# automl/TransformersCanDoBayesianInference

Hardware: AMD Instinct MI355X
Metric: synthetic datasets/sec (GP prior, bptt=2000) (higher is better)
Workload: dtype fp16; 1 GPU; priors.fast_gp, bptt=2000, num_features=18, emsize=512, nhead=4, nhid=1024, nlayers=6, 1000 bars (BASELINE.json configs[1]); per_gpu_batch=64, global_batch=64, aggregate_k_gradients=1, aggregate_streams=0, aggregate_stacked=False, seq_len=2000, parallelism=dp1, micro_batch_streams=2, eval_pos=weighted sampler(2000)

## Files before the change

### include/pfn_hip.h

```cpp
#ifndef PFN_HIP_H
#define PFN_HIP_H

#include <stddef.h>
#include <stdint.h>

#ifdef __cplusplus
extern "C" {
#endif

#define PFN_ABI_VERSION 10

enum {
  PFN_OK = 0,
  PFN_ERR_UNSUPPORTED = -1,
  PFN_ERR_ALIGNMENT = -2,
  PFN_ERR_LAUNCH = -3,
  PFN_ERR_ARGUMENT = -4,
};

enum { PFN_PREC_BF16 = 0,
       PFN_PREC_F32 = 1,
       PFN_PREC_FP16 = 2   };

typedef struct pfn_model_desc {
// ... 24 lines not shown
       PFN_TUNE_GEMM_TN_WRAP = 1,
       PFN_TUNE_FUSE_LNBWD = 2,
       PFN_TUNE_ATTN_PINGPONG = 4,
       PFN_TUNE_FUSE_LN_WIDE = 5,
       PFN_TUNE_GP_PLANES = 8,
       PFN_TUNE_FUSE_DELTA = 9,
       PFN_TUNE_GEMM_LN_ROWS = 7,
       PFN_TUNE_ATTN_BWD_GROUP = 10,
       PFN_TUNE_WGRAD_SPLITS = 11,
       PFN_TUNE_WGRAD_WAVES = 14,
       PFN_TUNE_LOSS_SCALE_TARGET = 15,
       PFN_TUNE_RESIDUAL16 = 16,
       PFN_TUNE_FUSE_Q_PROJECTION = 12,
       PFN_TUNE_KEY_CENTERING = 13,
       PFN_TUNE_ATTN_CACHE_SPLITS = 17,
       PFN_TUNE_TOP_LAYER_TEST_ROWS = 6  };
int pfn_set_tuning(int key, int value);
enum { PFN_PROF_ATTN_FWD = 0, PFN_PROF_ATTN_BWD_DELTA = 2, PFN_PROF_ATTN_BWD_KV = 4, PFN_PROF_ATTN_BWD_DQ = 6, PFN_PROF_GEMM_QKV = 8,
       PFN_PROF_GEMM_OUT_LN = 10, PFN_PROF_GEMM_LIN1 = 12, PFN_PROF_GEMM_LIN2_LN = 14, PFN_PROF_GEMM_DHPRE = 16, PFN_PROF_GEMM_DY1 = 18,
       PFN_PROF_GEMM_DCTX = 20, PFN_PROF_GEMM_DX = 22, PFN_PROF_WGRAD = 24, PFN_PROF_SLOTS = 26 };
int pfn_profile_enable(int on);
int pfn_profile_read(int slot, double* total_ms, int64_t* launches);

int pfn_param_layout(const pfn_model_desc* d, int64_t* offsets, int64_t* numels, int max_tensors);
int64_t pfn_param_count(const pfn_model_desc* d);
int64_t pfn_shadow_bytes(const pfn_model_desc* d);
int pfn_prepare_params(const pfn_model_desc* d, const float* params, void* shadow, void* stream);

int64_t pfn_workspace_bytes(const pfn_model_desc* d, int B, int S);
int64_t pfn_top_layer_rows(const pfn_model_desc* d, int B, int S, int sep, int use_dropout);
// ... 157 lines not shown
                      float* value, float* grad, void* stream);
int pfn_bnn_predict(const float* x_test, const float* theta, int64_t ld, int P, int K, int m, int F, int H, int activation,
                    float* prob1, void* stream);

int pfn_mlp_prior_forward(const float* weights, const float* biases, const int32_t* model_of, const int32_t* dims,
                          const float* noise_std, float* causes, const float* noise, float* y, float* hidden,
                          int B, int T, int HP, int Lmax, int activation, int gen_causes,
                          uint64_t seed, uint64_t offset, void* stream);

int pfn_op_gemm_nt(const void* A, int64_t lda, const void* B, int64_t ldb, int M, int N, int K,
                   int flags, const float* bias, const void* aux, int64_t ld_aux,
                   const float* resid, int64_t ld_resid, float* out_f32, int64_t ld_out_f32,
                   void* out_t, int64_t ld_out_t, void* out2_t, int64_t ld_out2, int prec, void* stream);
int pfn_op_gemm_tn(const void* A, int64_t lda, const void* B, int64_t ldb, float* C, int64_t ldc,
                   int M, int P, int Q, int atomic, int prec, void* stream);
int pfn_op_gemm_tn_group(int n, const void* const* A, const int64_t* lda, const void* const* B, const int64_t* ldb,
                         float* const* C, const int64_t* ldc, const int32_t* P, const int32_t* Q,
                         float* const* colsum, int M, int splits, int prec, void* stream);
#define PFN_OP_SUMS_16BIT 256
int pfn_op_gemm_ln(const void* A, int64_t lda, const void* B, int64_t ldb, int M, int N, int K, const float* bias,
                   const float* resid, const float* ry, const float* rmean, const float* rrstd,
                   const float* rgamma, const float* rbeta, const float* gamma, const float* beta, float eps,
                   float* y, float* mean, float* rstd, void* x_t, int prec, void* stream);
int pfn_op_gemm_lnbwd(const void* A, int64_t lda, const void* B, int64_t ldb, int M, int N, int K, const void* aux,
                      const float* y, const float* mean, const float* rstd, const float* gamma,
                      void* dx_t, float* dgamma, float* dbeta, int prec, void* stream);
int pfn_op_attention_fwd(const void* qkv, void* ctx, float* lse, int B, int S, int E, int H, int sep,
                         int prec, void* stream);
int64_t pfn_op_attention_bwd_ws_bytes(int B, int S, int H, int prec);
int pfn_op_attention_bwd(const void* qkv, const void* ctx, const float* lse, const void* dctx,
// ... 23 lines not shown
```

### transformerscandobayesianinference_amd/_hip.py

```python
import ctypes
import os
import subprocess

import torch

_HERE = os.path.dirname(os.path.abspath(__file__))
LIB_PATH = os.path.join(_HERE, 'libpfn_hip.so')
ABI_VERSION = 10

MAX_FEATURES = 1022
PREC_BF16 = 0
PREC_F32 = 1
PREC_FP16 = 2
PRECISIONS = {'bf16': PREC_BF16, 'f32': PREC_F32, 'fp32': PREC_F32, 'fp16': PREC_FP16, 'f16': PREC_FP16}
SCHED_TOP_LAYER_ALL_ROWS, SCHED_FUSE_LN_WIDE, SCHED_SEPARATE_LNBWD, SCHED_DETERMINISTIC, SCHED_NO_KEY_CENTERING, SCHED_FUSE_Q_PROJECTION, SCHED_KEY_CENTERING, SCHED_F32_RESIDUAL = 1, 2, 4, 8, 16, 32, 64, 128
NUTS_ADAPT_MASS, NUTS_KEEP_WARMUP, NUTS_MAX_WINDOWS, NUTS_INV_MASS_OFFSET = 1, 2, 16, 256

EPI_BIAS, EPI_GELU, EPI_GELU_BWD, EPI_RESID, EPI_OUT_F32, EPI_OUT_T, EPI_OUT2_T, EPI_ACCUM, EPI_RESID_T = 1, 2, 4, 8, 16, 32, 64, 128, 256


class HipExtensionError(RuntimeError):
    pass


# ... 55 lines not shown
    'pfn_clip_adam_step': (_I, [_P, _P, _P, _P, _L, _F, _F, _F, _F, _F, _F, _I, _I, _P, _P]),
    'pfn_gp_workspace_bytes': (_L, [_I, _I]),
    'pfn_gp_prior_sample': (_I, [_P, _P, _P, _P, _L, _P, _P, _P, _I, _I, _I, _I, _I, _I, _U64, _U64, _P, _P]),
    'pfn_gp_posterior': (_I, [_P, _P, _P, _L, _P, _P, _P, _P, _P, _I, _I, _I, _I, _P, _P, _P, _P, _P]),
    'pfn_gp_fit_workspace_bytes': (_L, [_I, _I]),
    'pfn_gp_mll_grad': (_I, [_P, _P, _P, _P, _P, _I, _I, _I, _I, _I, _P, _L, _P, _P, _P, _P]),
    'pfn_gp_fit_predict': (_I, [_P, _P, _P, _P, _P, _I, _I, _I, _I, _P, _I, _P, _L, _P, _P, _P, _P]),
    'pfn_nuts_workspace_bytes': (_L, [_I, _I, _I]),
    'pfn_nuts_init': (_I, [_P, _L, _I, _I, _L, _I, _I, _I, _I, _P, _I, _I, _F, _F, _U64, _P, _P, _P, _P, _P, _P]),
    'pfn_nuts_advance': (_I, [_P, _L, _I, _I, _L, _I, _I, _I, _P, _P, _P, _P, _P, _P, _P, _P, _P, _P, _P]),
    'pfn_bnn_logp_grad': (_I, [_P, _P, _P, _P, _L, _I, _I, _I, _I, _I, _I, _P, _P, _P]),
    'pfn_bnn_predict': (_I, [_P, _P, _L, _I, _I, _I, _I, _I, _I, _P, _P]),
    'pfn_mlp_prior_forward': (_I, [_P, _P, _P, _P, _P, _P, _P, _P, _P, _I, _I, _I, _I, _I, _I, _U64, _U64, _P]),
    'pfn_op_gemm_nt': (_I, [_P, _L, _P, _L, _I, _I, _I, _I, _P, _P, _L, _P, _L, _P, _L, _P, _L, _P, _L, _I, _P]),
    'pfn_op_gemm_tn': (_I, [_P, _L, _P, _L, _P, _L, _I, _I, _I, _I, _I, _P]),
    'pfn_op_gemm_tn_group': (_I, [_I, _P, _P, _P, _P, _P, _P, _P, _P, _P, _I, _I, _I, _P]),
    'pfn_op_gemm_ln': (_I, [_P, _L, _P, _L, _I, _I, _I, _P, _P, _P, _P, _P, _P, _P, _P, _P, _F, _P, _P, _P, _P, _I, _P]),
    'pfn_op_gemm_lnbwd': (_I, [_P, _L, _P, _L, _I, _I, _I, _P, _P, _P, _P, _P, _P, _P, _P, _I, _P]),
    'pfn_op_attention_fwd': (_I, [_P, _P, _P, _I, _I, _I, _I, _I, _I, _P]),
    'pfn_op_attention_bwd_ws_bytes': (_L, [_I, _I, _I, _I]),
    'pfn_op_attention_fwd_from': (_I, [_P, _P, _P, _I, _I, _I, _I, _I, _I, _I, _P]),
    'pfn_op_attention_bwd_from': (_I, [_P, _P, _P, _P, _P, _P, _P, _I, _I, _I, _I, _I, _I, _I, _I, _P]),
    'pfn_op_gather_rows': (_I, [_P, _P, _I, _I, _L, _I, _P]),
    'pfn_op_scatter_rows': (_I, [_P, _P, _I, _I, _L, _I, _I, _P]),
    'pfn_op_attention_bwd': (_I, [_P, _P, _P, _P, _P, _P, _P, _I, _I, _I, _I, _I, _I, _I, _P]),
    'pfn_op_layernorm_fwd': (_I, [_P, _P, _P, _P, _P, _P, _P, _L, _I, _F, _I, _P]),
    'pfn_op_layernorm_bwd': (_I, [_P, _I, _P, _P, _P, _P, _P, _P, _P, _P, _P, _L, _I, _I, _P]),
    'pfn_op_cast': (_I, [_P, _P, _L, _I, _P]),
    'pfn_op_qkv_projection': (_I, [_P, _P, _P, _P, _P, _I, _I, _I, _I, _P, _I, _I, _P]),
}
# ... 54 lines not shown
```

### transformerscandobayesianinference_amd/csrc/gemm_tn.hip

```cpp
#include <type_traits>
#include "pfn_device.h"
#include "pfn_kernels.h"

namespace pfn {

PFN_DEV int xcd_remap(int bid, int nwg) {
  const int q = nwg >> 3, r = nwg & 7, xcd = bid & 7;
  return (xcd < r ? xcd * (q + 1) : r * (q + 1) + (xcd - r) * q) + (bid >> 3);
}
typedef __attribute__((address_space(1))) const void gvoid_t;
typedef __attribute__((address_space(3))) void lvoid_t;

constexpr int TN_BMK = 32;

template <typename T>
__global__ __launch_bounds__(256, 2) void gemm_tn_kernel(GemmTN g) {
  constexpr int RB = 128 * sizeof(T);
  constexpr int TILE = TN_BMK * RB;
  extern __shared__ __attribute__((aligned(16))) char smem_raw[];
  LdsPtr smem = lds_cast(smem_raw);
  auto tileA = [&](int buf) { return smem + buf * 2 * TILE; };
  auto tileB = [&](int buf) { return smem + buf * 2 * TILE + TILE; };

  const int p0 = blockIdx.y * 128, q0 = blockIdx.x * 128;
// ... 473 lines not shown
#else
    return PFN_ERR_UNSUPPORTED;
#endif
  }
  static LdsAllowance allowance[2];
  if (precision == PFN_PREC_FP16) {
    allowance[1].ensure(gemm_tn_big_kernel<f16>, TNB_LDS);
    hipLaunchKernelGGL(gemm_tn_big_kernel<f16>, dim3(tiles * splits), dim3(512), TNB_LDS, stream, g);
  } else {
    allowance[0].ensure(gemm_tn_big_kernel<bf16>, TNB_LDS);
    hipLaunchKernelGGL(gemm_tn_big_kernel<bf16>, dim3(tiles * splits), dim3(512), TNB_LDS, stream, g);
  }
  return hipGetLastError() == hipSuccess ? PFN_OK : PFN_ERR_LAUNCH;
}

}
```

### transformerscandobayesianinference_amd/csrc/pfn_api.hip

```cpp
#include <algorithm>
#include <cstdarg>
#include <cstdio>
#include <cstring>
#include <mutex>
#include <vector>
#include "pfn_kernels.h"

using namespace pfn;

namespace pfn {
namespace {
struct ProfPair { hipEvent_t a, b; };
std::mutex g_prof_mu;
std::vector<ProfPair> g_prof[PFN_PROF_SLOTS];
std::atomic<int> g_prof_on{0};
}
bool prof_enabled() { return g_prof_on.load(std::memory_order_relaxed) != 0; }
void* prof_begin(int slot, hipStream_t s) {
  const int on = g_prof_on.load(std::memory_order_relaxed);
  if (!on || slot < 0 || slot >= PFN_PROF_SLOTS) return nullptr;
  if (on >= 2 && (slot & ~1) != on - 2) return nullptr;
  ProfPair* p = new ProfPair;
  if (hipEventCreate(&p->a) != hipSuccess || hipEventCreate(&p->b) != hipSuccess) { delete p; return nullptr; }
  (void)hipEventRecord(p->a, s);
// ... 93 lines not shown
  float* x0; char* x0_t;
  char* xaug_t;
  float* embacc;
  float* xaug_amax;
  std::vector<LayerWs> layer;
  char *xt_t, *dpre, *dt;
  char *dlog_t, *dd_t, *dctx_t;
  float *dxt, *gA, *delta;
  char* ds;
  char* gA_t;
  char *top_ctx_t, *top_dy1_t, *top_dctx_t;
  float *top_ry, *top_rmean, *top_rrstd;
  float* kshift;
  float* lscale;
  float* ln_part;
  int64_t bytes;
};

struct Ragged { const int32_t* sep_of; const int64_t* row_off; int64_t test_rows; int sep_min; };

static bool key_centering(const pfn_model_desc& d) {
  return (d.precision == PFN_PREC_FP16 && !(d.schedule & PFN_SCHED_NO_KEY_CENTERING)) || (d.precision == PFN_PREC_BF16 && (d.schedule & PFN_SCHED_KEY_CENTERING));
}

static bool residual16(const pfn_model_desc& d) {
  const int E = d.emsize;
  const bool wide = (d.schedule & PFN_SCHED_FUSE_LN_WIDE) != 0;
  return d.precision == PFN_PREC_FP16 && !(d.schedule & PFN_SCHED_F32_RESIDUAL) && d.nlayers > 0 && d.dropout == 0.f && d.nhid % 32 == 0 &&
         (E == 128 || E == 256 || E == 512 || (E == 1024 && wide));
}
static bool residual16_separate_ln(const pfn_model_desc& d, bool ln_fusable) {
  return d.precision == PFN_PREC_FP16 && !(d.schedule & PFN_SCHED_F32_RESIDUAL) && d.nlayers > 0 && d.dropout == 0.f && d.emsize >= 1024 && d.emsize % 8 == 0 && !ln_fusable;
}

Ws carve(const pfn_model_desc& d, int B, int S, char* base) {
  Ws w;
  const int64_t M = (int64_t)B * S, E = d.emsize, F = d.nhid, es = esize(d.precision);
  const int64_t npad = align_up(d.n_out, 8);
  int64_t cur = 0;
  auto take = [&](int64_t nbytes) { char* p = base ? base + cur : nullptr; cur = align_up(cur + nbytes, 256); return p; };
  w.x0 = (float*)take(M * E * 4); w.x0_t = take(M * E * es);
  const int64_t aug = emb_aug_width(d.num_features) > 0 ? emb_aug_width(d.num_features) : 32;
  w.xaug_t = take(M * aug * es); w.embacc = (float*)take(E * aug * 4);
  w.xaug_amax = (float*)take(aug * 4);
  w.layer.resize(d.nlayers);
  for (auto& l : w.layer) {
    l.qkv = take(M * 3 * E * es); l.ctx = take(M * E * es); l.lse = (float*)take((int64_t)B * d.nhead * S * 4);
    l.y1 = (float*)take(M * E * 4); l.mean1 = (float*)take(M * 4); l.rstd1 = (float*)take(M * 4);
    l.x1 = (float*)take(M * E * 4); l.x1_t = take(M * E * es);
// ... 4 lines not shown
    l.dy2m_t = l.dy1m_t = nullptr;
    if (d.dropout > 0.f) { l.dy2m_t = take(M * E * es); l.dy1m_t = take(M * E * es); }
  }
  w.xt_t = take(M * E * es); w.dpre = take(M * F * es); w.dt = take(M * F * es);
  w.dlog_t = take(M * npad * es); w.dd_t = take(M * F * es); w.dxt = (float*)take(M * E * 4);
  w.gA = (float*)take(M * E * 4); w.gA_t = take(M * E * es);
  w.dctx_t = take(M * E * es);
  w.delta = (float*)take(2 * (int64_t)B * d.nhead * S * 4);
  w.ds = take(attn_bwd_ds_bytes(B, S, d.nhead, d.precision));
  const int64_t Mtop = (d.nlayers > 0 && d.dropout == 0.f && !(d.schedule & PFN_SCHED_TOP_LAYER_ALL_ROWS)) ? (int64_t)B * (S - (S + 3) / 4) : 0;
  w.top_ctx_t = take(Mtop * E * es); w.top_dy1_t = take(Mtop * E * es); w.top_dctx_t = take(Mtop * E * es);
  w.top_ry = (float*)take(Mtop * E * 4); w.top_rmean = (float*)take(Mtop * 4); w.top_rrstd = (float*)take(Mtop * 4);
  w.kshift = key_centering(d) ? (float*)take((int64_t)B * E * 4) : nullptr;
  w.lscale = (float*)take(256);
  w.ln_part = (d.schedule & PFN_SCHED_DETERMINISTIC) ? (float*)take((int64_t)LNB_MAX_BLOCKS * 3 * E * 4) : nullptr;
  w.bytes = cur;
  return w;
}

struct Context { int64_t kv_bytes, shift_bytes, layer_bytes, bytes; };
static bool context_centred(const pfn_model_desc& d) { return key_centering(d) && d.emsize % 64 == 0; }
Context context_layout(const pfn_model_desc& d, int B, int sep) {
  Context c;
  c.kv_bytes = align_up((int64_t)B * sep * 2 * d.emsize * esize(d.precision), 256);
  c.shift_bytes = context_centred(d) ? align_up((int64_t)B * d.emsize * 4, 256) : 0;
  c.layer_bytes = sep > 0 ? c.kv_bytes + c.shift_bytes : 0;
  c.bytes = c.layer_bytes * d.nlayers;
  return c;
}
struct KvSink { char* base; Context c; };
// ... 102 lines not shown
  const int E = d.emsize, sched = d.schedule;
  const bool width_ok = (E <= 512 || (sched & PFN_SCHED_FUSE_LN_WIDE));
  pl.ln_ok = ln_gemm_probe(d, x0, x0_t, params, sh, M);
  const bool ln_fusable = pl.ln_ok && d.nhid % 32 == 0 && width_ok;
  pl.fuse_ln = prec_is16(d.precision) && ln_fusable && pdrop == 0.f;
  pl.y16 = residual16(d) && pl.ln_ok;
  pl.y16u = residual16_separate_ln(d, ln_fusable);
  pl.y16_any = pl.y16 || pl.y16u;
  pl.lnb_eligible = !(sched & PFN_SCHED_DETERMINISTIC) && !(sched & PFN_SCHED_SEPARATE_LNBWD) && prec_is16(d.precision) && d.nlayers > 0 && pdrop == 0.f && width_ok;
  return pl;
}

bool emb_gemm(const pfn_model_desc& d, bool custom_encoder) {
  return !custom_encoder && prec_is16(d.precision) && d.nlayers > 0 && emb_aug_width(d.num_features) > 0 && d.emsize % 8 == 0;
}
bool predict_dsrc_is_t(const pfn_model_desc& d) { return d.nlayers > 0 && prec_is16(d.precision); }

struct Resid { const float* plain; const void* y; const float* mean; const float* rstd; const float* gamma; const float* beta; };
void set_resid(GemmLN& g, const Resid& r) { g.resid = r.plain; g.ry = r.y; g.rmean = r.mean; g.rrstd = r.rstd; g.rgamma = r.gamma; g.rbeta = r.beta; }
struct LayerBufs { const float* xin; const char* xin_t; char *qkv, *ctx; float* lse; float *y1, *mean1, *rstd1, *x1; char *x1_t, *h, *hpre; float *y2, *mean2, *rstd2, *x2; char* x2_t; };

int layer_tail_forward(const Model& m, const LayerP& p, const LayerBufs& u, Resid& res, int rows, const Plan& pl, float pdrop, const unsigned* seed, bool last, int prof) {
  const pfn_model_desc& d = *m.d;
  const int prec = d.precision, E = d.emsize, F = d.nhid;
  const float* params = m.params;
  hipStream_t s = m.s;
  const bool y16u = pl.y16u;
  if (pl.fuse_ln) {
    ProfScope ps(PFN_PROF_GEMM_OUT_LN + prof, s);
    GemmLN g; memset(&g, 0, sizeof(g));
// ... 143 lines not shown
  }
  if (fuse_lnb) {
    ProfScope ps(PFN_PROF_GEMM_DY1 + prof, s);
    PFN_TRY(launch_gemm_lnbwd(lnb_dy1(m, pl, lsc, t, g, rows), prec, s));
  } else {
    {
      GemmNT gm = nt(g.dh_t, F, WT(m, t.w1), F, rows, E, F, EPI_RESID_T | EPI_OUT_T);
      gm.aux = g.dy2_t; gm.ld_aux = E; gm.out_t = g.dx1_t; gm.ld_out_t = E;
      PFN_TRY(launch_gemm_nt(gm, prec, s));
    }
    PFN_TRY(launch_layernorm_bwd(g.dx1_t, 1, g.y1, g.gamma1, g.mean1, g.rstd1, nullptr, g.dy1_t, g.ln1.dgamma, g.ln1.dbeta, g.ln1.dbias, rows, E, prec, s,
                                 g.ln_part, lsc, pl.y16_any));
  }
  return PFN_OK;
}
int layer_backward_dx(const Model& m, const LayerP& t, const char* dqkv_t, const char* dy1_t, int rows, const Plan& pl, const float* lsc, const LayerGrads* below,
                      float* gA, char* gA_t, bool out_f32, int prof) {
  const int prec = m.d->precision, E = m.d->emsize;
  if (below) {
    ProfScope ps(PFN_PROF_GEMM_DX + prof, m.s);
    return launch_gemm_lnbwd(lnb_dx(m, pl, lsc, t, dqkv_t, dy1_t, *below, rows), prec, m.s);
  }
  GemmNT g = nt(dqkv_t, 3 * E, WT(m, t.w_in), 3 * E, rows, E, 3 * E, EPI_RESID_T | (out_f32 ? EPI_OUT_F32 : EPI_OUT_T));
  g.aux = dy1_t; g.ld_aux = E; g.out_f32 = gA; g.ld_out_f32 = E; g.out_t = gA_t; g.ld_out_t = E;
  return launch_gemm_nt(g, prec, m.s);
}

}

extern "C" {

static bool g_gp_planes = true;
static bool g_fuse_delta = true;
static int g_default_schedule = 0;
static bool top_layer_on_test_rows(const pfn_model_desc& d, int S, int sep, float pdrop) {
  return !(d.schedule & PFN_SCHED_TOP_LAYER_ALL_ROWS) && d.nlayers > 0 && pdrop == 0.f && d.dropout == 0.f && sep < S && 4L * sep >= S;
}
static bool top_layer_on_test_rows_ragged(const pfn_model_desc& d, int S, const Ragged& rg, float pdrop) {
  return !(d.schedule & PFN_SCHED_TOP_LAYER_ALL_ROWS) && d.nlayers > 0 && pdrop == 0.f && d.dropout == 0.f && rg.test_rows > 0 && 4L * rg.sep_min >= S;
}
// ... 27 lines not shown
    case PFN_TUNE_ATTN_BWD_GROUP: set_attn_bwd_group(value); return PFN_OK;
    case PFN_TUNE_WGRAD_SPLITS: set_gemm_tn_group_splits(value); return PFN_OK;
    case PFN_TUNE_WGRAD_WAVES: set_gemm_tn_group_waves(value); return PFN_OK;
    case PFN_TUNE_LOSS_SCALE_TARGET: return set_loss_scale_target(value);
    case PFN_TUNE_RESIDUAL16: g_default_schedule = value ? (g_default_schedule & ~PFN_SCHED_F32_RESIDUAL) : (g_default_schedule | PFN_SCHED_F32_RESIDUAL); return PFN_OK;
    case PFN_TUNE_FUSE_Q_PROJECTION: g_default_schedule = value ? (g_default_schedule | PFN_SCHED_FUSE_Q_PROJECTION) : (g_default_schedule & ~PFN_SCHED_FUSE_Q_PROJECTION); return PFN_OK;
    case PFN_TUNE_KEY_CENTERING:
      g_default_schedule &= ~(PFN_SCHED_NO_KEY_CENTERING | PFN_SCHED_KEY_CENTERING);
      if (value > 0) g_default_schedule |= PFN_SCHED_KEY_CENTERING; else if (value == 0) g_default_schedule |= PFN_SCHED_NO_KEY_CENTERING;
      return PFN_OK;
    case PFN_TUNE_GEMM_LN_ROWS: set_gemm_ln_rows64(value); return PFN_OK;
    case PFN_TUNE_GP_PLANES: g_gp_planes = value != 0; return PFN_OK;
    case PFN_TUNE_FUSE_DELTA: g_fuse_delta = value != 0; return PFN_OK;
    case PFN_TUNE_ATTN_CACHE_SPLITS: set_attn_cache_split_cap(value); return PFN_OK;
    case PFN_TUNE_FUSE_LN_WIDE: g_default_schedule = value ? (g_default_schedule | PFN_SCHED_FUSE_LN_WIDE) : (g_default_schedule & ~PFN_SCHED_FUSE_LN_WIDE); return PFN_OK;
    case PFN_TUNE_TOP_LAYER_TEST_ROWS: g_default_schedule = value ? (g_default_schedule & ~PFN_SCHED_TOP_LAYER_ALL_ROWS) : (g_default_schedule | PFN_SCHED_TOP_LAYER_ALL_ROWS); return PFN_OK;
    default: return fail(PFN_ERR_ARGUMENT, "unknown tuning key %d", key);
  }
}
const char* pfn_last_error_string(void) { return g_err; }

int pfn_param_layout(const pfn_model_desc* d, int64_t* offsets, int64_t* numels, int max_tensors) {
  int rc = check_desc(d);
  if (rc != PFN_OK) return rc;
  Layout L = make_layout(*d);
  const int n = (int)L.offsets.size();
  if (offsets || numels) {
    if (max_tensors < n) return fail(PFN_ERR_ARGUMENT, "need room for %d tensors, got %d", n, max_tensors);
    for (int i = 0; i < n; ++i) { if (offsets) offsets[i] = L.offsets[i]; if (numels) numels[i] = L.numels[i]; }
  }
// ... 492 lines not shown
    PFN_TRY(launch_tn_set(dec_grouped ? dec : std::vector<TnProblem>{dp0}, Mt, prec, det, lsc, NO_PROF, s, dec_grouped));
  }
  if (top_mode) {}
  else if (rg) PFN_TRY(launch_scatter_test_rows_ragged(dxt, d->nlayers > 0 ? (void*)w.gA_t : (void*)w.gA, S, B, E, rg->sep_of, (const long*)rg->row_off, d->nlayers > 0 ? prec : PFN_PREC_F32, s));
  else PFN_TRY(launch_scatter_test_rows(dxt, d->nlayers > 0 ? (void*)w.gA_t : (void*)w.gA, S, B, E, sep, d->nlayers > 0 ? prec : PFN_PREC_F32, s));

  auto view = [&](int l, bool compact) {
    const LayerP& p = L.layer[l];
    LayerWs& a = w.layer[l];
    float *db2 = pdrop > 0.f ? nullptr : grads + p.b2, *dbo = pdrop > 0.f ? nullptr : grads + p.b_o;
    return LayerGrads{compact ? (const void*)dxt : (const void*)w.gA_t, compact ? 0 : 1, a.y2, a.mean2, a.rstd2, params + p.g2, a.y1, a.mean1, a.rstd1, params + p.g1, a.hpre,
                      a.dy2_t, a.dy2m_t, a.dh_t, compact ? w.top_dy1_t : a.dy1_t, a.dqkv_t, w.gA_t,
                      LnSinks{grads + p.g2, grads + p.be2, db2}, LnSinks{grads + p.g1, grads + p.be1, dbo}, w.ln_part};
  };
  const bool emb_t = emb_gemm(*d, dsrc_sbe != nullptr);
  const bool fuse_lnb = d->nlayers > 0 && lnbwd_fusable(m, pl, lsc, view(0, false), M);
  auto launch_weight_gradients = [&](int l_hi, int l_lo) -> int {
    std::vector<TnProblem> probs, probs_top;
    auto add = [&](const void* A, long lda, const void* Bm, long ldb, float* C, long ldc, int P, int Q, float* colsum, bool compact = false) {
      TnProblem t; memset(&t, 0, sizeof(t)); t.A = A; t.lda = lda; t.B = Bm; t.ldb = ldb; t.C = C; t.ldc = ldc; t.P = P; t.Q = Q; t.colsum = colsum;
      (compact ? probs_top : probs).push_back(t);
    };
    for (int l = l_hi; l >= l_lo; --l) {
      const LayerP& p = L.layer[l];
      LayerWs& a = w.layer[l];
      const char* xin_t = (l == 0) ? w.x0_t : w.layer[l - 1].x2_t;
      const bool drop = pdrop > 0.f;
      const bool top = top_mode && l == d->nlayers - 1;
      add(drop ? a.dy2m_t : a.dy2_t, E, a.h, F, grads + p.w2, F, E, F, (drop || (fuse_lnb && l < d->nlayers - 1)) ? grads + p.b2 : nullptr, top);
      add(a.dh_t, F, a.x1_t, E, grads + p.w1, E, F, E, grads + p.b1, top);
// ... 41 lines not shown
        PFN_TRY(launch_scatter_rows(w.top_dy1_t, a.dy1_t, S, B, (long)E * es, sep, 0, s));
      }
    }
    {
      AttnArgs at; memset(&at, 0, sizeof(at));
      at.qkv = a.qkv; at.ctx = a.ctx; at.lse = a.lse; at.B = B; at.S = S; at.E = E; at.H = H; at.sep = sep; at.sep_of = sep_of;
      at.dctx = w.dctx_t; at.dqkv = a.dqkv_t; at.delta = w.delta; at.ds = w.ds;
      at.p_drop = pdrop; at.drop_seed = dseed(l, 0);
      at.q_begin = top ? (rg ? rg->sep_min : sep) : 0;
      at.q_from_sep = (top && rg) ? 1 : 0;
      if (delta_fused) at.parts = ATTN_BWD_KV | ATTN_BWD_DQ;
      at.zero_delta = delta_zeroed ? 1 : 0;
      PFN_TRY(launch_attn_bwd(at, prec, s));
    }
    const LayerGrads below = l > 0 ? view(l - 1, false) : LayerGrads{};
    PFN_TRY(layer_backward_dx(m, t, a.dqkv_t, a.dy1_t, M, pl, lsc, fuse_lnb && l > 0 ? &below : nullptr, w.gA, w.gA_t, l == 0 && !emb_t, 0));
    if (l == split_at) {
      PFN_TRY(launch_weight_gradients(d->nlayers - 1, split_at));
      on_first_group(user);
    }
  }
  if (d->nlayers > 0) PFN_TRY(launch_weight_gradients(split_at >= 0 ? split_at - 1 : d->nlayers - 1, 0));
  const int aug = emb_aug_width(d->num_features);
  if (dsrc_sbe) {
    PFN_TRY(launch_bse_to_sbe(w.gA, dsrc_sbe, S, B, E, s, lsc));
  } else if (emb_t) {
    if (hipMemsetAsync(w.embacc, 0, sizeof(float) * E * aug, s) != hipSuccess) return fail(PFN_ERR_LAUNCH, "memset");
    GemmTN g = tn(w.gA_t, E, w.xaug_t, aug, w.embacc, aug, M, E, aug, grads + L.enc_b);
    g.scale_amax = lsc;
    g.max_splits = det ? 1 : 128;
    PFN_TRY(launch_gemm_tn(g, prec, s));
    PFN_TRY(launch_embed_grad_scatter(w.embacc, grads + L.enc_w, grads + L.yenc_w, grads + L.yenc_b, E, d->num_features, prec == PFN_PREC_FP16 ? w.xaug_amax : nullptr, s));
  } else {
    EmbedBwdArgs e;
    e.dsrc = w.gA; e.x = x; e.x_st = x_st; e.x_sb = x_sb; e.y = y; e.y_st = y_st; e.y_sb = y_sb;
    e.dwx = grads + L.enc_w; e.dbx = grads + L.enc_b; e.dwy = grads + L.yenc_w; e.dby = grads + L.yenc_b;
    e.S = S; e.B = B; e.nf = d->num_features; e.E = E; e.sep = sep; e.sep_of = sep_of; e.single_block = det ? 1 : 0; e.scale_amax = lsc;
    PFN_TRY(launch_embed_bwd(e, s));
  }
  return PFN_OK;
}

int pfn_stack_input_grads(const pfn_model_desc* d, const float* params, int B, int S, int sep, const void* workspace, int64_t workspace_bytes,
                          float* dx, int64_t dx_st, int64_t dx_sb, float* dy, int64_t dy_st, int64_t dy_sb, void* stream) {
  PFN_TRY(check_desc(d));
  if (B < 1 || S < 1 || sep < 0 || sep > S) return fail(PFN_ERR_ARGUMENT, "bad B=%d S=%d sep=%d", B, S, sep);
  if (!params || !workspace || !dx) return fail(PFN_ERR_ARGUMENT, "null pointer");
  Ws w = carve(*d, B, S, (char*)workspace);
  if (workspace_bytes < w.bytes) return fail(PFN_ERR_ARGUMENT, "workspace too small: %lld < %lld", (long long)workspace_bytes, (long long)w.bytes);
  const int prec = d->precision, E = d->emsize;
  const Layout L = make_layout(*d);
  hipStream_t s = (hipStream_t)stream;
  const bool emb_t = emb_gemm(*d, false);
  EmbedInGradArgs e; memset(&e, 0, sizeof(e));
  e.dsrc = emb_t ? (const void*)w.gA_t : (const void*)w.gA; e.dsrc_prec = emb_t ? prec : PFN_PREC_F32;
  e.wx = params + L.enc_w; e.wy = params + L.yenc_w;
  e.dx = dx; e.dx_st = dx_st; e.dx_sb = dx_sb; e.dy = dy; e.dy_st = dy_st; e.dy_sb = dy_sb;
  e.S = S; e.B = B; e.nf = d->num_features; e.E = E; e.sep = sep;
  e.scale_amax = (prec == PFN_PREC_FP16 && sep < S) ? w.lscale : nullptr;
  return launch_embed_input_grad(e, s);
}

int pfn_bar_mean_backward(const float* logits, int64_t ld, const float* borders, int64_t R, int nbars, int full_support, const float* mean, const float* gout,
                          float* dlogits, void* stream) {
  if (R < 0 || nbars < 1 || (R > 0 && (!logits || !borders || !mean || !gout || !dlogits))) return fail(PFN_ERR_ARGUMENT, "bad bar_mean_backward arguments");
  BarArgs a; memset(&a, 0, sizeof(a));
  a.logits = logits; a.ld = ld; a.borders = borders; a.R = R; a.nbars = nbars; a.full_support = full_support;
  a.mean_out = const_cast<float*>(mean); a.gout = gout; a.dlogits = dlogits;
// ... 243 lines not shown
int pfn_op_gemm_nt(const void* A, int64_t lda, const void* B, int64_t ldb, int M, int N, int K, int flags, const float* bias,
                   const void* aux, int64_t ld_aux, const float* resid, int64_t ld_resid, float* out_f32, int64_t ld_out_f32,
                   void* out_t, int64_t ld_out_t, void* out2_t, int64_t ld_out2, int prec, void* stream) {
  GemmNT g = nt(A, lda, B, ldb, M, N, K, flags);
  g.bias = bias; g.aux = aux; g.ld_aux = ld_aux; g.resid = resid; g.ld_resid = ld_resid; g.out_f32 = out_f32; g.ld_out_f32 = ld_out_f32;
  g.out_t = out_t; g.ld_out_t = ld_out_t; g.out2_t = out2_t; g.ld_out2 = ld_out2;
  PFN_TRY(launch_gemm_nt(g, prec, (hipStream_t)stream));
  return PFN_OK;
}
int pfn_op_gemm_tn(const void* A, int64_t lda, const void* B, int64_t ldb, float* C, int64_t ldc, int M, int P, int Q, int atomic, int prec, void* stream) {
  GemmTN g = tn(A, lda, B, ldb, C, ldc, M, P, Q);
  g.atomic = atomic;
  PFN_TRY(launch_gemm_tn(g, prec, (hipStream_t)stream));
  return PFN_OK;
}
int pfn_op_gemm_tn_group(int n, const void* const* A, const int64_t* lda, const void* const* B, const int64_t* ldb, float* const* C,
                         const int64_t* ldc, const int32_t* P, const int32_t* Q, float* const* colsum, int M, int splits, int prec, void* stream) {
  if (n < 1 || n > TN_GROUP_MAX || !A || !lda || !B || !ldb || !C || !ldc || !P || !Q) return fail(PFN_ERR_ARGUMENT, "bad gemm_tn_group arguments");
  GemmTNGroup g;
  memset(&g, 0, sizeof(g));
  g.n = n; g.M = M; g.splits = splits;
  for (int i = 0; i < n; ++i) {
    TnProblem& t = g.p[i];
    t.A = A[i]; t.lda = lda[i]; t.B = B[i]; t.ldb = ldb[i]; t.C = C[i]; t.ldc = ldc[i]; t.P = P[i]; t.Q = Q[i];
    t.colsum = colsum ? colsum[i] : nullptr;
  }
  PFN_TRY(launch_gemm_tn_group(g, prec, (hipStream_t)stream));
  return PFN_OK;
}
int pfn_op_gemm_ln(const void* A, int64_t lda, const void* B, int64_t ldb, int M, int N, int K, const float* bias,
// ... 92 lines not shown
```

### transformerscandobayesianinference_amd/csrc/pfn_kernels.h

```cpp
#pragma once
#include <hip/hip_runtime.h>
#include <stdint.h>
#include <atomic>
#include "../../include/pfn_hip.h"

namespace pfn {

struct LdsAllowance {
  std::atomic<size_t> granted[16];
  template <typename K> void ensure(K kernel, size_t bytes) {
    int dev = 0;
    (void)hipGetDevice(&dev);
    std::atomic<size_t>& g = granted[dev & 15];
    if (bytes <= g.load(std::memory_order_acquire)) return;
    (void)hipFuncSetAttribute(reinterpret_cast<const void*>(kernel), hipFuncAttributeMaxDynamicSharedMemorySize, (int)bytes);
    size_t cur = g.load(std::memory_order_relaxed);
    while (cur < bytes && !g.compare_exchange_weak(cur, bytes, std::memory_order_release)) {}
  }
};

inline bool prec_is16(int p) { return p == PFN_PREC_BF16 || p == PFN_PREC_FP16; }
inline int prec_esize(int p) { return prec_is16(p) ? 2 : 4; }
#define PFN_DISPATCH_OP(prec, ...)                                                          \
  do {                                                                                      \
// ... 67 lines not shown
void set_gemm_nt_big_mode(int mode);
void set_gemm_ln_rows64(int on);

struct GemmTN {
  const void* A; long lda;
  const void* B; long ldb;
  float* C; long ldc;
  int M, P, Q;
  int atomic;
  int m_chunk;
  float* colsum;
  int max_splits;
  const float* scale_amax;
};
int launch_gemm_tn(GemmTN g, int precision, hipStream_t stream);

constexpr int TN_GROUP_MAX = 26;
struct TnProblem {
  const void* A; const void* B; float* C; float* colsum;
  long lda, ldb, ldc;
  int P, Q;
  int Pv;
};
struct GemmTNGroup {
  TnProblem p[TN_GROUP_MAX];
  int tile_start[TN_GROUP_MAX + 1];
  int n, M, splits, m_chunk;
  int debug_mask;
  const float* scale_amax;
};
// ... 306 lines not shown
```

Before: 2589 datasets/s.

## Compute embedding gradients directly from layer-0 dqkv/dy1 instead of the dx GEMM

In the backward pass, layer 0 no longer runs its input-gradient GEMM (dqkv·W_in + dy1) to form gA. The embedding weight gradient is instead computed by reassociation: a skinny TN GEMM of dqkv and dy1 against the augmented input xaug (width 32-128) into a 4E×aug scratch, then a fold kernel multiplies by W_in and adds the dy1 part. This replaces an M×E×3E GEMM plus an M×E×aug GEMM with an M×4E×aug GEMM and a small fold. It adds atomics-based nondeterminism, so it is disabled under the deterministic schedule. Where the input gradient is still needed, it is recomputed from a transposed W_in copy.

```diff
diff --git a/include/pfn_hip.h b/include/pfn_hip.h
--- a/include/pfn_hip.h
+++ b/include/pfn_hip.h
@@ -62,6 +62,7 @@
        PFN_TUNE_FUSE_Q_PROJECTION = 12,
        PFN_TUNE_KEY_CENTERING = 13,
        PFN_TUNE_ATTN_CACHE_SPLITS = 17,
+       PFN_TUNE_EMBED_GRAD_DSRC = 18,
        PFN_TUNE_TOP_LAYER_TEST_ROWS = 6  };
 int pfn_set_tuning(int key, int value);
 enum { PFN_PROF_ATTN_FWD = 0, PFN_PROF_ATTN_BWD_DELTA = 2, PFN_PROF_ATTN_BWD_KV = 4, PFN_PROF_ATTN_BWD_DQ = 6, PFN_PROF_GEMM_QKV = 8,
@@ -249,6 +250,8 @@
                    void* out_t, int64_t ld_out_t, void* out2_t, int64_t ld_out2, int prec, void* stream);
 int pfn_op_gemm_tn(const void* A, int64_t lda, const void* B, int64_t ldb, float* C, int64_t ldc,
                    int M, int P, int Q, int atomic, int prec, void* stream);
+int pfn_op_embed_grad(const void* dqkv, const void* dy1, const void* xaug, const float* w_in, int M, int E, int aug,
+                      float* scratch, float* embacc, float* dbias, int splits, int prec, void* stream);
 int pfn_op_gemm_tn_group(int n, const void* const* A, const int64_t* lda, const void* const* B, const int64_t* ldb,
                          float* const* C, const int64_t* ldc, const int32_t* P, const int32_t* Q,
                          float* const* colsum, int M, int splits, int prec, void* stream);
diff --git a/transformerscandobayesianinference_amd/_hip.py b/transformerscandobayesianinference_amd/_hip.py
--- a/transformerscandobayesianinference_amd/_hip.py
+++ b/transformerscandobayesianinference_amd/_hip.py
@@ -93,6 +93,7 @@
     'pfn_mlp_prior_forward': (_I, [_P, _P, _P, _P, _P, _P, _P, _P, _P, _I, _I, _I, _I, _I, _I, _U64, _U64, _P]),
     'pfn_op_gemm_nt': (_I, [_P, _L, _P, _L, _I, _I, _I, _I, _P, _P, _L, _P, _L, _P, _L, _P, _L, _P, _L, _I, _P]),
     'pfn_op_gemm_tn': (_I, [_P, _L, _P, _L, _P, _L, _I, _I, _I, _I, _I, _P]),
+    'pfn_op_embed_grad': (_I, [_P, _P, _P, _P, _I, _I, _I, _P, _P, _P, _I, _I, _P]),
     'pfn_op_gemm_tn_group': (_I, [_I, _P, _P, _P, _P, _P, _P, _P, _P, _P, _I, _I, _I, _P]),
     'pfn_op_gemm_ln': (_I, [_P, _L, _P, _L, _I, _I, _I, _P, _P, _P, _P, _P, _P, _P, _P, _P, _F, _P, _P, _P, _P, _I, _P]),
     'pfn_op_gemm_lnbwd': (_I, [_P, _L, _P, _L, _I, _I, _I, _P, _P, _P, _P, _P, _P, _P, _P, _I, _P]),
diff --git a/transformerscandobayesianinference_amd/csrc/gemm_tn.hip b/transformerscandobayesianinference_amd/csrc/gemm_tn.hip
--- a/transformerscandobayesianinference_amd/csrc/gemm_tn.hip
+++ b/transformerscandobayesianinference_amd/csrc/gemm_tn.hip
@@ -511,4 +511,191 @@
   return hipGetLastError() == hipSuccess ? PFN_OK : PFN_ERR_LAUNCH;
 }
 
-}
+#ifndef PFN_SKINNY_KT
+#define PFN_SKINNY_KT 64
+#endif
+constexpr int SKINNY_KT = PFN_SKINNY_KT;
+template <typename T, int NQ, int KT>
+__global__ __launch_bounds__(256) void gemm_tn_skinny_kernel(GemmTNSkinny g) {
+  static_assert(sizeof(T) == 2, "16-bit operands");
+  constexpr int RBA = 256 * sizeof(T), RBB = 32 * NQ * sizeof(T);
+  constexpr int TILEA = KT * RBA, TILEB = KT * RBB;
+  extern __shared__ __attribute__((aligned(16))) char smem_raw[];
+  LdsPtr smem = lds_cast(smem_raw);
+  auto tileA = [&](int buf) { return smem + buf * (TILEA + TILEB); };
+  auto tileB = [&](int buf) { return smem + buf * (TILEA + TILEB) + TILEA; };
+
+  const bool second = (int)blockIdx.x >= g.tiles0;
+  const int P = second ? g.P1 : g.P0;
+  const long lda = second ? g.lda1 : g.lda0;
+  const int p0 = (second ? (int)blockIdx.x - g.tiles0 : (int)blockIdx.x) * 256;
+  const int grow0 = second ? g.P0 : 0;
+  const int colsA = min(256, P - p0);
+  const long mbeg = (long)blockIdx.y * g.m_chunk;
+  const long mend = min((long)g.M, mbeg + g.m_chunk);
+  if (mbeg >= mend) return;
+  const T* A = reinterpret_cast<const T*>(second ? g.A1 : g.A0) + mbeg * lda + p0;
+  const T* B = reinterpret_cast<const T*>(g.B) + mbeg * g.ldb;
+
+  const int wave = threadIdx.x >> 6, lane = threadIdx.x & 63;
+
+  f32x16 acc[2][NQ];
+#pragma unroll
+  for (int i = 0; i < 2; ++i)
+#pragma unroll
+    for (int j = 0; j < NQ; ++j)
+#pragma unroll
+      for (int r = 0; r < 16; ++r) acc[i][j][r] = 0.f;
+
+  TileStage<T, KT, RBA, 256> sa;
+  TileStage<T, KT, RBB, 256> sb;
+  const int rows_total = (int)(mend - mbeg);
+  const int nt = (rows_total + KT - 1) / KT;
+  float csum[8];
+#pragma unroll
+  for (int e = 0; e < 8; ++e) csum[e] = 0.f;
+  auto add_colsum = [&]() {
+#pragma unroll
+    for (int i = 0; i < sa.PER; ++i) {
+      const X8<T> v = __builtin_bit_cast(X8<T>, sa.regs[i]);
+#pragma unroll
+      for (int e = 0; e < 8; ++e) csum[e] += (float)v[e];
+    }
+  };
+  sa.issue(A, lda, rows_total, colsA);
+  sb.issue(B, g.ldb, rows_total, g.Q);
+  add_colsum();
+  sa.template commit<true>(tileA(0));
+  sb.template commit<true>(tileB(0));
+  __syncthreads();
+  for (int t = 0; t < nt; ++t) {
+    const int cur = t & 1;
+    if (t + 1 < nt) {
+      const long r1 = (long)(t + 1) * KT;
+      sa.issue(A + r1 * lda, lda, rows_total - (int)r1, colsA);
+      sb.issue(B + r1 * g.ldb, g.ldb, rows_total - (int)r1, g.Q);
+      add_colsum();
+    }
+    const lds_char* ta = tileA(cur);
+    const lds_char* tb = tileB(cur);
+#pragma unroll
+    for (int ks = 0; ks < KT; ks += 16) {
+      Frag<T> fa[2], fb[NQ];
+#pragma unroll
+      for (int i = 0; i < 2; ++i) fa[i] = load_frag_tr<T, RBA, 1>(ta, ks, wave * 64 + i * 32);
+#pragma unroll
+      for (int j = 0; j < NQ; ++j) fb[j] = load_frag_tr<T, RBB, 1>(tb, ks, j * 32);
+#pragma unroll
+      for (int i = 0; i < 2; ++i)
+#pragma unroll
+        for (int j = 0; j < NQ; ++j) acc[i][j] = mma32(fa[i], fb[j], acc[i][j]);
+    }
+    if (t + 1 < nt) {
+      sa.template commit<true>(tileA(cur ^ 1));
+      sb.template commit<true>(tileB(cur ^ 1));
+    }
+    __syncthreads();
+  }
+
+  const float osc = loss_scale_down(g.scale_amax);
+  {
+    constexpr int NCH = RBA / 16;
+    float* red = reinterpret_cast<float*>(smem_raw);
+#pragma unroll
+    for (int e = 0; e < 8; ++e) red[threadIdx.x * 8 + e] = csum[e];
+    __syncthreads();
+    if (threadIdx.x < NCH) {
+#pragma unroll
+      for (int e = 0; e < 8; ++e) {
+        float t = 0.f;
+        for (int j = 0; j < 256 / NCH; ++j) t += red[(j * NCH + threadIdx.x) * 8 + e];
+        const int col = p0 + threadIdx.x * 8 + e;
+        if (col < P) unsafeAtomicAdd(g.gsum + grow0 + col, t * osc);
+      }
+    }
+  }
+#pragma unroll
+  for (int i = 0; i < 2; ++i)
+#pragma unroll
+    for (int j = 0; j < NQ; ++j)
+#pragma unroll
+      for (int r = 0; r < 16; ++r) {
+        const int p = p0 + wave * 64 + i * 32 + acc_row(r, lane);
+        const int q = j * 32 + (lane & 31);
+        if (p < P && q < g.Q) unsafeAtomicAdd(g.G + (long)(grow0 + p) * g.Q + q, acc[i][j][r] * osc);
+      }
+}
+
+template <typename T, int NQ> static void launch_skinny_t(const GemmTNSkinny& g, dim3 grid, hipStream_t stream) {
+  const size_t lds = 2 * SKINNY_KT * (256 + 32 * NQ) * 2;
+  static LdsAllowance allowance;
+  allowance.ensure(gemm_tn_skinny_kernel<T, NQ, SKINNY_KT>, lds);
+  hipLaunchKernelGGL((gemm_tn_skinny_kernel<T, NQ, SKINNY_KT>), grid, dim3(256), lds, stream, g);
+}
+int launch_gemm_tn_skinny(GemmTNSkinny g, int precision, hipStream_t stream) {
+  if (g.M <= 0 || g.P0 + g.P1 <= 0) return PFN_OK;
+  if (!prec_is16(precision) || (g.Q != 32 && g.Q != 64 && g.Q != 128) || g.P0 < 0 || g.P1 < 0) return PFN_ERR_UNSUPPORTED;
+  if ((g.lda0 * 2) % 16 || (g.lda1 * 2) % 16 || (g.ldb * 2) % 16 || !aligned16(g.A0) || !aligned16(g.A1) || !aligned16(g.B)) return PFN_ERR_ALIGNMENT;
+  g.tiles0 = (g.P0 + 255) / 256;
+  const int tiles = g.tiles0 + (g.P1 + 255) / 256;
+  int splits = g.splits > 0 ? g.splits : (512 + tiles - 1) / tiles;
+  const int max_splits = (g.M + 4 * SKINNY_KT - 1) / (4 * SKINNY_KT);
+  if (splits > max_splits) splits = max_splits;
+  if (splits > 65535) splits = 65535;
+  if (splits < 1) splits = 1;
+  int chunk = (g.M + splits - 1) / splits;
+  chunk = (chunk + SKINNY_KT - 1) / SKINNY_KT * SKINNY_KT;
+  splits = (g.M + chunk - 1) / chunk;
+  g.m_chunk = chunk;
+  const dim3 grid(tiles, splits);
+  if (precision == PFN_PREC_FP16) {
+    if (g.Q == 32) launch_skinny_t<f16, 1>(g, grid, stream); else if (g.Q == 64) launch_skinny_t<f16, 2>(g, grid, stream); else launch_skinny_t<f16, 4>(g, grid, stream);
+  } else {
+    if (g.Q == 32) launch_skinny_t<bf16, 1>(g, grid, stream); else if (g.Q == 64) launch_skinny_t<bf16, 2>(g, grid, stream); else launch_skinny_t<bf16, 4>(g, grid, stream);
+  }
+  return hipGetLastError() == hipSuccess ? PFN_OK : PFN_ERR_LAUNCH;
+}
+
+constexpr int FOLD_J = 64;
+__global__ __launch_bounds__(256) void embed_grad_fold_kernel(const float* __restrict__ G, const float* __restrict__ gsum, const float* __restrict__ w_in,
+                                                              float* embacc, float* dbias, int E, int aug) {
+  const int e = blockIdx.x * 32 + (threadIdx.x & 31), sl = threadIdx.x >> 5;
+  if (e >= E) return;
+  const int n4 = aug / 32;
+  const int a0 = sl * (aug / 8);
+  const int j0 = blockIdx.y * FOLD_J, j1 = min(3 * E, j0 + FOLD_J);
+  f32x4 acc[4];
+#pragma unroll
+  for (int k = 0; k < 4; ++k) acc[k] = f32x4{0.f, 0.f, 0.f, 0.f};
+  float bs = 0.f;
+  for (int j = j0; j < j1; ++j) {
+    const float w = w_in[(long)j * E + e];
+    const f32x4* row = reinterpret_cast<const f32x4*>(G + (long)j * aug + a0);
+#pragma unroll
+    for (int k = 0; k < 4; ++k)
+      if (k < n4) acc[k] += w * row[k];
+    if (sl == 0) bs += w * gsum[j];
+  }
+  if (blockIdx.y == 0) {
+    const f32x4* row = reinterpret_cast<const f32x4*>(G + (long)(3 * E + e) * aug + a0);
+#pragma unroll
+    for (int k = 0; k < 4; ++k)
+      if (k < n4) acc[k] += row[k];
+    if (sl == 0) bs += gsum[3 * E + e];
+  }
+#pragma unroll
+  for (int k = 0; k < 4; ++k)
+    if (k < n4) {
+#pragma unroll
+      for (int c = 0; c < 4; ++c) unsafeAtomicAdd(embacc + (long)e * aug + a0 + 4 * k + c, acc[k][c]);
+    }
+  if (sl == 0) unsafeAtomicAdd(dbias + e, bs);
+}
+int launch_embed_grad_fold(const float* G, const float* gsum, const float* w_in, float* embacc, float* dbias, int E, int aug, hipStream_t stream) {
+  if ((aug != 32 && aug != 64 && aug != 128) || !aligned16(G)) return PFN_ERR_UNSUPPORTED;
+  const dim3 grid((E + 31) / 32, (3 * E + FOLD_J - 1) / FOLD_J);
+  hipLaunchKernelGGL(embed_grad_fold_kernel, grid, dim3(256), 0, stream, G, gsum, w_in, embacc, dbias, E, aug);
+  return hipGetLastError() == hipSuccess ? PFN_OK : PFN_ERR_LAUNCH;
+}
+
+}
diff --git a/transformerscandobayesianinference_amd/csrc/pfn_api.hip b/transformerscandobayesianinference_amd/csrc/pfn_api.hip
--- a/transformerscandobayesianinference_amd/csrc/pfn_api.hip
+++ b/transformerscandobayesianinference_amd/csrc/pfn_api.hip
@@ -131,6 +131,8 @@
   float* kshift;
   float* lscale;
   float* ln_part;
+  float* emb_g;
+  char* win_t;
   int64_t bytes;
 };
 
@@ -150,6 +152,7 @@
   return d.precision == PFN_PREC_FP16 && !(d.schedule & PFN_SCHED_F32_RESIDUAL) && d.nlayers > 0 && d.dropout == 0.f && d.emsize >= 1024 && d.emsize % 8 == 0 && !ln_fusable;
 }
 
+inline int64_t emb_g_floats(int64_t E, int64_t aug) { return 4 * E * aug + 4 * E + E * aug; }
 Ws carve(const pfn_model_desc& d, int B, int S, char* base) {
   Ws w;
   const int64_t M = (int64_t)B * S, E = d.emsize, F = d.nhid, es = esize(d.precision);
@@ -184,6 +187,8 @@
   w.kshift = key_centering(d) ? (float*)take((int64_t)B * E * 4) : nullptr;
   w.lscale = (float*)take(256);
   w.ln_part = (d.schedule & PFN_SCHED_DETERMINISTIC) ? (float*)take((int64_t)LNB_MAX_BLOCKS * 3 * E * 4) : nullptr;
+  w.emb_g = (float*)take(emb_g_floats(E, aug) * 4);
+  w.win_t = take(3 * E * E * es);
   w.bytes = cur;
   return w;
 }
@@ -316,6 +321,10 @@
 bool emb_gemm(const pfn_model_desc& d, bool custom_encoder) {
   return !custom_encoder && prec_is16(d.precision) && d.nlayers > 0 && emb_aug_width(d.num_features) > 0 && d.emsize % 8 == 0;
 }
+static bool g_embed_grad_dsrc = false;
+bool embed_grad_direct(const pfn_model_desc& d, bool custom_encoder) {
+  return emb_gemm(d, custom_encoder) && !(d.schedule & PFN_SCHED_DETERMINISTIC) && !g_embed_grad_dsrc;
+}
 bool predict_dsrc_is_t(const pfn_model_desc& d) { return d.nlayers > 0 && prec_is16(d.precision); }
 
 struct Resid { const float* plain; const void* y; const float* mean; const float* rstd; const float* gamma; const float* beta; };
@@ -489,6 +498,11 @@
   }
   return PFN_OK;
 }
+int plain_dx(int prec, int E, const char* dqkv_t, const char* dy1_t, const void* win_t, int rows, float* gA, char* gA_t, bool out_f32, hipStream_t s) {
+  GemmNT g = nt(dqkv_t, 3 * E, win_t, 3 * E, rows, E, 3 * E, EPI_RESID_T | (out_f32 ? EPI_OUT_F32 : EPI_OUT_T));
+  g.aux = dy1_t; g.ld_aux = E; g.out_f32 = gA; g.ld_out_f32 = E; g.out_t = gA_t; g.ld_out_t = E;
+  return launch_gemm_nt(g, prec, s);
+}
 int layer_backward_dx(const Model& m, const LayerP& t, const char* dqkv_t, const char* dy1_t, int rows, const Plan& pl, const float* lsc, const LayerGrads* below,
                       float* gA, char* gA_t, bool out_f32, int prof) {
   const int prec = m.d->precision, E = m.d->emsize;
@@ -496,9 +510,7 @@
     ProfScope ps(PFN_PROF_GEMM_DX + prof, m.s);
     return launch_gemm_lnbwd(lnb_dx(m, pl, lsc, t, dqkv_t, dy1_t, *below, rows), prec, m.s);
   }
-  GemmNT g = nt(dqkv_t, 3 * E, WT(m, t.w_in), 3 * E, rows, E, 3 * E, EPI_RESID_T | (out_f32 ? EPI_OUT_F32 : EPI_OUT_T));
-  g.aux = dy1_t; g.ld_aux = E; g.out_f32 = gA; g.ld_out_f32 = E; g.out_t = gA_t; g.ld_out_t = E;
-  return launch_gemm_nt(g, prec, m.s);
+  return plain_dx(prec, E, dqkv_t, dy1_t, WT(m, t.w_in), rows, gA, gA_t, out_f32, m.s);
 }
 
 }
@@ -556,6 +568,7 @@
     case PFN_TUNE_FUSE_DELTA: g_fuse_delta = value != 0; return PFN_OK;
     case PFN_TUNE_ATTN_CACHE_SPLITS: set_attn_cache_split_cap(value); return PFN_OK;
     case PFN_TUNE_FUSE_LN_WIDE: g_default_schedule = value ? (g_default_schedule | PFN_SCHED_FUSE_LN_WIDE) : (g_default_schedule & ~PFN_SCHED_FUSE_LN_WIDE); return PFN_OK;
+    case PFN_TUNE_EMBED_GRAD_DSRC: g_embed_grad_dsrc = value != 0; return PFN_OK;
     case PFN_TUNE_TOP_LAYER_TEST_ROWS: g_default_schedule = value ? (g_default_schedule & ~PFN_SCHED_TOP_LAYER_ALL_ROWS) : (g_default_schedule | PFN_SCHED_TOP_LAYER_ALL_ROWS); return PFN_OK;
     default: return fail(PFN_ERR_ARGUMENT, "unknown tuning key %d", key);
   }
@@ -1078,6 +1091,7 @@
                       LnSinks{grads + p.g2, grads + p.be2, db2}, LnSinks{grads + p.g1, grads + p.be1, dbo}, w.ln_part};
   };
   const bool emb_t = emb_gemm(*d, dsrc_sbe != nullptr);
+  const bool emb_direct = embed_grad_direct(*d, dsrc_sbe != nullptr);
   const bool fuse_lnb = d->nlayers > 0 && lnbwd_fusable(m, pl, lsc, view(0, false), M);
   auto launch_weight_gradients = [&](int l_hi, int l_lo) -> int {
     std::vector<TnProblem> probs, probs_top;
@@ -1149,7 +1163,7 @@
       PFN_TRY(launch_attn_bwd(at, prec, s));
     }
     const LayerGrads below = l > 0 ? view(l - 1, false) : LayerGrads{};
-    PFN_TRY(layer_backward_dx(m, t, a.dqkv_t, a.dy1_t, M, pl, lsc, fuse_lnb && l > 0 ? &below : nullptr, w.gA, w.gA_t, l == 0 && !emb_t, 0));
+    if (l > 0 || !emb_direct) PFN_TRY(layer_backward_dx(m, t, a.dqkv_t, a.dy1_t, M, pl, lsc, fuse_lnb && l > 0 ? &below : nullptr, w.gA, w.gA_t, l == 0 && !emb_t, 0));
     if (l == split_at) {
       PFN_TRY(launch_weight_gradients(d->nlayers - 1, split_at));
       on_first_group(user);
@@ -1159,6 +1173,15 @@
   const int aug = emb_aug_width(d->num_features);
   if (dsrc_sbe) {
     PFN_TRY(launch_bse_to_sbe(w.gA, dsrc_sbe, S, B, E, s, lsc));
+  } else if (emb_direct) {
+    float *G = w.emb_g, *gsum = G + 4L * E * aug, *acc = gsum + 4L * E;
+    if (hipMemsetAsync(G, 0, sizeof(float) * emb_g_floats(E, aug), s) != hipSuccess) return fail(PFN_ERR_LAUNCH, "memset");
+    GemmTNSkinny g; memset(&g, 0, sizeof(g));
+    g.A0 = w.layer[0].dqkv_t; g.lda0 = 3 * E; g.P0 = 3 * E; g.A1 = w.layer[0].dy1_t; g.lda1 = E; g.P1 = E;
+    g.B = w.xaug_t; g.ldb = aug; g.Q = aug; g.G = G; g.gsum = gsum; g.M = M; g.scale_amax = lsc;
+    PFN_TRY(launch_gemm_tn_skinny(g, prec, s));
+    PFN_TRY(launch_embed_grad_fold(G, gsum, params + L.layer[0].w_in, acc, grads + L.enc_b, E, aug, s));
+    PFN_TRY(launch_embed_grad_scatter(acc, grads + L.enc_w, grads + L.yenc_w, grads + L.yenc_b, E, d->num_features, prec == PFN_PREC_FP16 ? w.xaug_amax : nullptr, s));
   } else if (emb_t) {
     if (hipMemsetAsync(w.embacc, 0, sizeof(float) * E * aug, s) != hipSuccess) return fail(PFN_ERR_LAUNCH, "memset");
     GemmTN g = tn(w.gA_t, E, w.xaug_t, aug, w.embacc, aug, M, E, aug, grads + L.enc_b);
@@ -1187,6 +1210,11 @@
   const Layout L = make_layout(*d);
   hipStream_t s = (hipStream_t)stream;
   const bool emb_t = emb_gemm(*d, false);
+  if (embed_grad_direct(*d, false)) {
+    const LayerWs& a = w.layer[0];
+    PFN_TRY(launch_transpose_cast(params + L.layer[0].w_in, w.win_t, 3 * E, E, 3 * E, prec, s));
+    PFN_TRY(plain_dx(prec, E, a.dqkv_t, a.dy1_t, w.win_t, B * S, w.gA, w.gA_t, false, s));
+  }
   EmbedInGradArgs e; memset(&e, 0, sizeof(e));
   e.dsrc = emb_t ? (const void*)w.gA_t : (const void*)w.gA; e.dsrc_prec = emb_t ? prec : PFN_PREC_F32;
   e.wx = params + L.enc_w; e.wy = params + L.yenc_w;
@@ -1460,6 +1488,19 @@
   PFN_TRY(launch_gemm_tn(g, prec, (hipStream_t)stream));
   return PFN_OK;
 }
+int pfn_op_embed_grad(const void* dqkv, const void* dy1, const void* xaug, const float* w_in, int M, int E, int aug, float* scratch, float* embacc, float* dbias,
+                      int splits, int prec, void* stream) {
+  if (!dqkv || !dy1 || !xaug || !w_in || !scratch || !embacc || !dbias || M < 1 || E < 8 || E % 8) return fail(PFN_ERR_ARGUMENT, "bad embed_grad arguments");
+  hipStream_t s = (hipStream_t)stream;
+  float* gsum = scratch + 4L * E * aug;
+  if (hipMemsetAsync(scratch, 0, sizeof(float) * 4L * E * (aug + 1), s) != hipSuccess || hipMemsetAsync(embacc, 0, sizeof(float) * E * aug, s) != hipSuccess)
+    return fail(PFN_ERR_LAUNCH, "memset");
+  GemmTNSkinny g; memset(&g, 0, sizeof(g));
+  g.A0 = dqkv; g.lda0 = 3 * E; g.P0 = 3 * E; g.A1 = dy1; g.lda1 = E; g.P1 = E; g.B = xaug; g.ldb = aug; g.Q = aug; g.G = scratch; g.gsum = gsum; g.M = M; g.splits = splits;
+  PFN_TRY(launch_gemm_tn_skinny(g, prec, s));
+  PFN_TRY(launch_embed_grad_fold(scratch, gsum, w_in, embacc, dbias, E, aug, s));
+  return PFN_OK;
+}
 int pfn_op_gemm_tn_group(int n, const void* const* A, const int64_t* lda, const void* const* B, const int64_t* ldb, float* const* C,
                          const int64_t* ldc, const int32_t* P, const int32_t* Q, float* const* colsum, int M, int splits, int prec, void* stream) {
   if (n < 1 || n > TN_GROUP_MAX || !A || !lda || !B || !ldb || !C || !ldc || !P || !Q) return fail(PFN_ERR_ARGUMENT, "bad gemm_tn_group arguments");
diff --git a/transformerscandobayesianinference_amd/csrc/pfn_kernels.h b/transformerscandobayesianinference_amd/csrc/pfn_kernels.h
--- a/transformerscandobayesianinference_amd/csrc/pfn_kernels.h
+++ b/transformerscandobayesianinference_amd/csrc/pfn_kernels.h
@@ -105,6 +105,19 @@
   const float* scale_amax;
 };
 int launch_gemm_tn(GemmTN g, int precision, hipStream_t stream);
+
+struct GemmTNSkinny {
+  const void* A0; long lda0; int P0;
+  const void* A1; long lda1; int P1;
+  const void* B; long ldb; int Q;
+  float* G; float* gsum;
+  int M;
+  int splits;
+  int m_chunk, tiles0;
+  const float* scale_amax;
+};
+int launch_gemm_tn_skinny(GemmTNSkinny g, int precision, hipStream_t stream);
+int launch_embed_grad_fold(const float* G, const float* gsum, const float* w_in, float* embacc, float* dbias, int E, int aug, hipStream_t stream);
 
 constexpr int TN_GROUP_MAX = 26;
 struct TnProblem {
```

After: 2591 datasets/s (median of 2 runs). No clear change (+0.0%).
